# pkusys/Auncel

Measured on AMD Instinct MI355X. Metric: queries/sec @ recall@10>=0.95, SIFT-10M d=128 IVF4096, 1/2/4/8 GPU, higher is better.
Workload: dtype u8

## Files before the change

auncel_amd/build.py:

```python
import os
import subprocess

HERE = os.path.dirname(os.path.abspath(__file__))
CSRC = os.path.join(HERE, "csrc")
LIBDIR = os.path.join(HERE, "lib")
LIB = os.path.join(LIBDIR, "libauncel_amd.so")
SOURCES = ["ivf_kernels.hip", "ivf_select.hip", "ivf_filter.hip", "dataset_io.cpp", "ivf_plan.hip", "ivf_kmeans.hip", "ivf_update.hip", "ivf_subset.hip", "ivf_selector.hip", "ivf_exact.hip", "ivf_reconstruct.hip", "ivf_engine.hip"]
FLAGS = ["--offload-arch=gfx950", "-O3", "-ffp-contract=off", "-std=c++17", "-fPIC", "-shared", "-Wno-unused-result"]


LAST = {"compiled": [], "reused": 0}


def _deps(src):
    hdrs = [os.path.join(CSRC, f) for f in os.listdir(CSRC) if f.endswith(".h")]
    return [os.path.join(CSRC, src)] + hdrs + [os.path.join(HERE, "..", "include", "auncel_amd.h")]


def build(force=False):
    from concurrent.futures import ThreadPoolExecutor
    extra = os.environ.get("AUNCEL_AMD_CXXFLAGS", "").split()
    stamp = os.path.join(LIBDIR, "flags.txt")
    want = " ".join(FLAGS + extra)
    same_flags = os.path.exists(stamp) and open(stamp).read() == want
    os.makedirs(LIBDIR, exist_ok=True)
    objdir = os.path.join(LIBDIR, "obj")
    os.makedirs(objdir, exist_ok=True)
    hipcc = os.environ.get("HIPCC", "/opt/rocm/bin/hipcc")
    cflags = [f for f in FLAGS if f != "-shared"]
    todo = []
    for s in SOURCES:
        o = os.path.join(objdir, s + ".o")
        stale = force or not same_flags or not os.path.exists(o) or any(os.path.getmtime(p) > os.path.getmtime(o) for p in _deps(s))
        if stale:
            todo.append([hipcc] + cflags + extra + ["-c", os.path.join(CSRC, s), "-o", o])
    LAST["compiled"], LAST["reused"] = [os.path.basename(c[-3]) for c in todo], len(SOURCES) - len(todo)
    if not todo and os.path.exists(LIB) and same_flags:
        return LIB
    with ThreadPoolExecutor(max_workers=len(SOURCES)) as ex:
        for r in ex.map(lambda c: subprocess.run(c), todo):
            if r.returncode != 0:
                raise RuntimeError("hipcc failed")
    objs = [os.path.join(objdir, s + ".o") for s in SOURCES]
    subprocess.run([hipcc, "--offload-arch=gfx950", "-shared", "-fPIC"] + objs + ["-o", LIB], check=True)
    with open(stamp, "w") as f:
        f.write(want)
    return LIB


HOST_LIB = os.path.join(LIBDIR, "libfaiss_amd.so")
HOST_DIR = os.path.join(CSRC, "host")


def build_host(force=False):
    build(force)
    srcs = [os.path.join(HOST_DIR, f) for f in os.listdir(HOST_DIR)]
    if not force and os.path.exists(HOST_LIB) and all(os.path.getmtime(p) <= os.path.getmtime(HOST_LIB) for p in srcs + [LIB]):
        return HOST_LIB
    cmd = ["g++", "-std=c++17", "-O2", "-fPIC", "-shared", os.path.join(HOST_DIR, "faiss_amd.cpp"), "-o", HOST_LIB,
           "-L" + LIBDIR, "-launcel_amd", "-Wl,-rpath,$ORIGIN", "-pthread"]
    subprocess.run(cmd, check=True)
    return HOST_LIB


if __name__ == "__main__":
    print(build(force=True))
    print(build_host(force=True))
```

auncel_amd/csrc/ivf_engine.hip:

```cpp
#include <hip/hip_runtime.h>

#include <algorithm>
#include <atomic>
#include <cfloat>
#include <cmath>
#include <cstdlib>
#include <chrono>
#include <condition_variable>
#include <deque>
#include <functional>
#include <map>
#include <cstring>
#include <memory>
#include <stdexcept>
#include <string>
#include <mutex>
#include <thread>
#include <unordered_set>
#include <vector>

#include "../../include/auncel_amd.h"
#include "exact_args.h"
#include "ivf_kernels.h"
#include "kmeans_host.h"
// ... 1581 lines not shown
void coarse_dev(amd_ivf* h, const float* d_x, size_t n, size_t nprobe, int mode, float* d_out_dis, int64_t* d_out_keys, int fused,
                size_t prefix = 0) {
    if (!ix(h)->have_centroids) throw EngineError("quantizer has no centroids");
    const bool gemm = mode == 1 || (mode < 0 && !(n < 20 && h->d % 4 == 0));
    const size_t nlist = h->nlist;
    hipStream_t s = h->stream;
    if (!gemm && !h->in_coarse_pick && opt(h, OPT_COARSE_PICK, 2) != 0 && n >= 256 && nprobe <= 128 && nlist <= 4096 && nlist >= 4 * nprobe + 64 &&
        prefix == 0 && h->ties_override < 0 && n * nlist <= h->dist_budget_floats) {
        size_t t = h->timer.begin(CAT_COARSE, s);
        h->w_xnorms.ensure(n * sizeof(float));
        h->w_dist.ensure(n * nlist * sizeof(float));
        static const bool dbg_pick = getenv("AUNCEL_AMD_DEBUG_PICK") != nullptr;
        h->c_pick_flag.ensure((n + 1 + 8 + 8) * 4);
        h->p_pick.ensure((n + 1 + 8) * 4);
        HIP_CHECK(hipMemsetAsync(h->c_pick_flag.p, 0, 4, s));
        if (dbg_pick) HIP_CHECK(hipMemsetAsync(h->c_pick_flag.as<uint32_t>() + n + 1 + 8, 0, 32, s));
        launch_row_norms(d_x, n, h->dpad, h->w_xnorms.as<float>(), s);
        const FilterParams* prm = nullptr;
        if (opt(h, OPT_COARSE_PICK, 2) >= 2 && ix(h)->d_cinfo.p) {
            h->w_qinfo.ensure(16);
            h->w_fparams.ensure(2 * sizeof(FilterParams));
            HIP_CHECK(hipMemsetAsync(h->w_qinfo.p, 0, 16, s));
            launch_amax(d_x, n, h->dpad, h->w_qinfo.as<uint32_t>(), s);
            FilterParams* p = h->w_fparams.as<FilterParams>() + 1;
            launch_half_params(h->w_qinfo.as<uint32_t>(), ix(h)->d_cinfo.as<uint32_t>(), h->d, p, s);
            launch_coarse_gemm16(h->metric, d_x, ix(h)->d_centroids.as<float>(), h->w_xnorms.as<float>(), ix(h)->d_centroid_norms.as<float>(),
                                 (int)n, (int)nlist, h->dpad, h->w_dist.as<float>(), p, s);
            prm = p;
        } else {
            launch_coarse_gemm(h->metric, d_x, ix(h)->d_centroids.as<float>(), h->w_xnorms.as<float>(), ix(h)->d_centroid_norms.as<float>(),
                               (int)n, (int)nlist, h->dpad, h->w_dist.as<float>(), s);
        }
        launch_coarse_pick(h->metric, h->w_dist.as<float>(), d_x, ix(h)->d_centroids.as<float>(), h->w_xnorms.as<float>(), ix(h)->centroid_norm_max,
                           (uint32_t)n, (uint32_t)nlist, (uint32_t)nprobe, h->dpad, d_out_dis, d_out_keys, h->c_pick_flag.as<uint32_t>(),
                           h->c_pick_flag.as<uint32_t>() + 1, s, prm, dbg_pick ? h->c_pick_flag.as<uint32_t>() + n + 1 + 8 : nullptr);
        h->timer.end(t, s);
        CopySegs c{};
        c.src[0] = h->c_pick_flag.p;
        c.dst[0] = h->p_pick.dev();
        c.words[0] = (uint32_t)(n + 1);
        c.n = 1;
        launch_copy_segs(c, s);
        HIP_CHECK(stream_sync(s));
        const uint32_t m = h->p_pick.as<uint32_t>()[0];
        if (dbg_pick) {
            uint32_t why[5];
            HIP_CHECK(hipMemcpy(why, h->c_pick_flag.as<uint32_t>() + n + 1 + 8, sizeof(why), hipMemcpyDeviceToHost));
            fprintf(stderr, "[pick] %u of %zu rankings flagged: threshold/scale %u, too many candidates %u, too few %u, not finite %u, equal distances %u\n", m, n,
                    why[0], why[1], why[2], why[3], why[4]);
        }
        if (const uint32_t m_flagged = m) {
            const uint32_t m = (m_flagged + 7u) & ~7u;
            if (m != m_flagged) {
                uint32_t* list = h->p_pick.as<uint32_t>() + 1;
                for (uint32_t i = m_flagged; i < m; i++) list[i] = list[0];
                HIP_CHECK(hipMemcpyAsync(h->c_pick_flag.as<uint32_t>() + 1 + m_flagged, list + m_flagged, (m - m_flagged) * 4, hipMemcpyHostToDevice, s));
            }
            h->c_pick_x.ensure((size_t)m * h->dpad * sizeof(float));
            h->c_pick_dis.ensure((size_t)m * nprobe * 4);
            h->c_pick_keys.ensure((size_t)m * nprobe * 8);
            launch_gather_rows(d_x, h->c_pick_flag.as<uint32_t>() + 1, m, (uint32_t)h->dpad, h->c_pick_x.as<float>(), s);
            struct Guard {
                bool& f;
                ~Guard() { f = false; }
            } guard{h->in_coarse_pick};
            h->in_coarse_pick = true;
            coarse_dev(h, h->c_pick_x.as<float>(), m, nprobe, mode, h->c_pick_dis.as<float>(), h->c_pick_keys.as<int64_t>(), fused, 0);
            launch_scatter_rows(h->c_pick_dis.p, h->c_pick_flag.as<uint32_t>() + 1, m, (uint32_t)nprobe, d_out_dis, s);
            launch_scatter_rows(h->c_pick_keys.p, h->c_pick_flag.as<uint32_t>() + 1, m, (uint32_t)(2 * nprobe), d_out_keys, s);
        }
        h->coarse_picked = n - m;
        return;
    }
    h->coarse_picked = 0;
    const size_t chunk = std::max<size_t>(1, std::min<size_t>(n, h->dist_budget_floats / std::max<size_t>(nlist, 1)));
    const bool use_heap = nprobe <= 128;
    const int ties_opt = (int)opt(h, OPT_COARSE_TIES, -1);
    const bool heap_ties = !use_heap && (h->ties_override >= 0 ? h->ties_override == 1 : ties_opt == 1 || (ties_opt != 0 && n < 20));
    for (size_t c0 = 0; c0 < n; c0 += chunk) {
        const size_t m = std::min(chunk, n - c0);
        const uint32_t qg = scan_shape_of((uint32_t)std::min<size_t>(m, scan_qblock(false)));
        const uint32_t tv = scan_tile_vecs(qg);
        const size_t nitems = ((m + qg * SCAN_RQ - 1) / (qg * SCAN_RQ)) * ((nlist + tv - 1) / tv);
        const uint64_t csig = ((uint64_t)c0 << 40) ^ ((uint64_t)m << 20) ^ (uint64_t)nlist ^ ((uint64_t)qg << 60) ^ (use_heap ? 1ull << 59 : 0ull);
        const size_t ng = (m + SCAN_RQ - 1) / SCAN_RQ;
        const bool cached = h->coarse_sig_valid && h->coarse_sig == csig;
        if (!cached) {
            h->p_pair_query.ensure(m * 4);
            h->p_pair_out.ensure(m * 8);
            h->p_items.ensure(nitems * sizeof(ScanItem));
            h->p_group_p0.ensure(ng * 4);
            h->p_group_cnt.ensure(ng * 4);
            uint32_t* pq = h->p_pair_query.as<uint32_t>();
            uint64_t* po = h->p_pair_out.as<uint64_t>();
            ScanItem* items = h->p_items.as<ScanItem>();
            for (size_t i = 0; i < m; i++) {
                pq[i] = (uint32_t)(c0 + i);
                po[i] = (uint64_t)i * nlist;
            }
            size_t ni = 0;
            for (uint32_t vb = 0; vb < nlist; vb += tv)
                for (uint32_t qb = 0; qb < m; qb += qg * SCAN_RQ) {
                    ScanItem& it = items[ni++];
                    it.vec_base = vb;
                    it.nvec = std::min<uint32_t>(tv, (uint32_t)nlist - vb);
                    it.vec_off = vb;
                    it.pair_begin = qb;
                    it.npair = std::min<uint32_t>(qg * SCAN_RQ, (uint32_t)m - qb);
                    it.qg = qg;
                    it.qgroup = qb / SCAN_RQ;
                }
            for (size_t g = 0; g < ng; g++) {
                h->p_group_p0.as<uint32_t>()[g] = (uint32_t)(g * SCAN_RQ);
                h->p_group_cnt.as<uint32_t>()[g] = (uint32_t)std::min<size_t>(SCAN_RQ, m - g * SCAN_RQ);
            }
            h->c_pair_query.ensure(m * 4);
            h->c_pair_out.ensure(m * 8);
            h->c_items.ensure(nitems * sizeof(ScanItem));
            h->c_group_p0.ensure(ng * 4);
            h->c_group_cnt.ensure(ng * 4);
            HIP_CHECK(hipMemcpyAsync(h->c_pair_query.p, pq, m * 4, hipMemcpyHostToDevice, s));
            HIP_CHECK(hipMemcpyAsync(h->c_pair_out.p, po, m * 8, hipMemcpyHostToDevice, s));
            HIP_CHECK(hipMemcpyAsync(h->c_items.p, items, nitems * sizeof(ScanItem), hipMemcpyHostToDevice, s));
            HIP_CHECK(hipMemcpyAsync(h->c_group_p0.p, h->p_group_p0.p, ng * 4, hipMemcpyHostToDevice, s));
            HIP_CHECK(hipMemcpyAsync(h->c_group_cnt.p, h->p_group_cnt.p, ng * 4, hipMemcpyHostToDevice, s));
            h->coarse_sig_valid = false;
        }
        h->w_dist.ensure(m * nlist * sizeof(float));
        h->w_qtile.ensure(std::max<size_t>(ng, 1) * (size_t)h->dpad * SCAN_RQ * sizeof(float));
        launch_pack_queries(d_x, h->c_pair_query.as<uint32_t>(), h->c_group_p0.as<uint32_t>(), h->c_group_cnt.as<uint32_t>(), ng, h->dpad,
                            h->w_qtile.as<float>(), s);
        ScanArgs sa{};
        sa.qtile = h->w_qtile.as<float>();
        sa.codes = ix(h)->d_centroids.as<float>();
        sa.queries = d_x;
        sa.items = h->c_items.as<ScanItem>();
        sa.pair_query = h->c_pair_query.as<uint32_t>();
        sa.pair_out = h->c_pair_out.as<uint64_t>();
        sa.dist = h->w_dist.as<float>();
        sa.d = h->dpad;
        sa.metric = h->metric;
        sa.fused = fused;
        size_t t = h->timer.begin(CAT_COARSE, s);
        if (gemm) {
            h->w_xnorms.ensure(m * sizeof(float));
            launch_row_norms(d_x + c0 * h->dpad, m, h->dpad, h->w_xnorms.as<float>(), s);
            launch_coarse_gemm(h->metric, d_x + c0 * h->dpad, ix(h)->d_centroids.as<float>(), h->w_xnorms.as<float>(),
                               ix(h)->d_centroid_norms.as<float>(), (int)m, (int)nlist, h->dpad, h->w_dist.as<float>(), s);
        } else {
            size_t n_qg[4] = {0, 0, 0, 0};
            n_qg[scan_qg_class(qg)] = nitems;
            launch_scan(sa, n_qg, s);
        }
        if (use_heap) {
            const size_t k = nprobe;
            h->c_heap_val.ensure(m * k * 4);
            h->c_heap_ref.ensure(m * k * 8);
            h->c_stage.ensure(m * 4);
            h->c_nscan.ensure(m * 8);
            h->c_done.ensure(m * 4);
            h->c_seg_off.ensure(m * 8);
            h->c_seg_list.ensure(m * 4);
            h->c_seg_count.ensure(m * 4);
            constexpr size_t MISC_BYTES = STATS_ROWS * 4 * 8 + 8;
            h->w_misc.ensure(MISC_BYTES);
            if (!cached) {
                h->p_seg_off.ensure(m * 8);
                h->p_seg_list.ensure(m * 4);
                h->p_seg_count.ensure(m * 4);
                for (size_t i = 0; i < m; i++) {
                    h->p_seg_off.as<uint64_t>()[i] = (uint64_t)i * nlist;
                    h->p_seg_list.as<int32_t>()[i] = 0;
                    h->p_seg_count.as<uint32_t>()[i] = 1;
                }
                HIP_CHECK(hipMemcpyAsync(h->c_seg_off.p, h->p_seg_off.p, m * 8, hipMemcpyHostToDevice, s));
                HIP_CHECK(hipMemcpyAsync(h->c_seg_list.p, h->p_seg_list.p, m * 4, hipMemcpyHostToDevice, s));
                HIP_CHECK(hipMemcpyAsync(h->c_seg_count.p, h->p_seg_count.p, m * 4, hipMemcpyHostToDevice, s));
            }
            launch_fill_f32(h->c_heap_val.as<float>(), m * k, h->metric == METRIC_L2 ? FLT_MAX : -FLT_MAX, s);
            launch_fill_i64(h->c_heap_ref.as<int64_t>(), m * k, -1, s);
            HIP_CHECK(hipMemsetAsync(h->c_stage.p, 0, m * 4, s));
            HIP_CHECK(hipMemsetAsync(h->c_nscan.p, 0, m * 8, s));
            HIP_CHECK(hipMemsetAsync(h->c_done.p, 0, m * 4, s));
            HIP_CHECK(hipMemsetAsync(h->w_misc.p, 0, MISC_BYTES, s));
            ReplayArgs ra{};
            ra.metric = h->metric;
            ra.k = (int)k;
            ra.nlist = (uint32_t)nlist;
            ra.nq = (uint32_t)m;
            ra.round_probes = 1;
            ra.dist = h->w_dist.as<float>();
            ra.seg_off = h->c_seg_off.as<uint64_t>();
            ra.seg_list = h->c_seg_list.as<int32_t>();
            ra.seg_count = h->c_seg_count.as<uint32_t>();
            ra.identity_ids = 1;
            ra.finalize_all = 1;
            ra.heap_val = h->c_heap_val.as<float>();
            ra.heap_ref = h->c_heap_ref.as<int64_t>();
            ra.stage = h->c_stage.as<uint32_t>();
            ra.nscan = h->c_nscan.as<unsigned long long>();
            ra.done = h->c_done.as<uint32_t>();
            ra.D = d_out_dis + c0 * nprobe;
            ra.I = d_out_keys + c0 * nprobe;
            ra.stats = h->w_misc.as<unsigned long long>();
            ra.error = reinterpret_cast<uint32_t*>(h->w_misc.as<unsigned long long>() + STATS_ROWS * 4);
            launch_replay(ra, s);
        } else {
            bool tail_neutral = false;
            if (sort_rows_ranks_a_prefix((uint32_t)nlist, (uint32_t)nprobe, (uint32_t)prefix) && c0 == 0 && m == n && d_out_dis == h->w_cdis.p &&
                d_out_keys == h->w_ckeys.p) {
                amd_ivf::CoarseTail& ct = h->coarse_tail;
                tail_neutral = ct.valid && ct.dis == d_out_dis && ct.keys == d_out_keys && ct.prefix == prefix && ct.nprobe == nprobe && ct.rows >= n &&
                               ct.metric == h->metric && ct.touch_dis + 1 == h->w_cdis.touch && ct.touch_keys + 1 == h->w_ckeys.touch &&
                               !getenv("AUNCEL_AMD_WRITE_TAILS");
                ct = amd_ivf::CoarseTail{true, d_out_dis, d_out_keys, prefix, nprobe, tail_neutral ? ct.rows : n, h->metric, h->w_cdis.touch, h->w_ckeys.touch};
            } else {
                h->coarse_tail.valid = false;
            }
            launch_sort_rows(h->w_dist.as<float>(), (uint32_t)m, (uint32_t)nlist, (uint32_t)nprobe, h->metric,
                             d_out_dis + c0 * nprobe, d_out_keys + c0 * nprobe, s, (uint32_t)prefix, tail_neutral);
            if (heap_ties) {
                if (!h->w_tie_rows.p) {
                    h->w_tie_rows.ensure(8);
                    HIP_CHECK(hipMemsetAsync(h->w_tie_rows.p, 0, 8, s));
                }
                const size_t nout = prefix && prefix < nprobe ? prefix : nprobe;
                const bool ran = launch_heap_tie_order(h->w_dist.as<float>(), (uint32_t)m, (uint32_t)nlist, (uint32_t)nprobe, (uint32_t)nout,
                                                       h->metric, d_out_dis + c0 * nprobe, d_out_keys + c0 * nprobe,
                                                       h->w_tie_rows.as<unsigned long long>(), s);
                if (!ran && (h->ties_override == 1 || ties_opt == 1))
                    throw EngineError("coarse tie order by the reference's heap needs nlist x 12 bytes of LDS (nlist <= ~13 000)");
            }
        }
        h->timer.end(t, s);
        if (!cached || c0 + m < n) {
            HIP_CHECK(stream_sync(s));
            if (c0 == 0 && m == n) {
                h->coarse_sig = csig;
                h->coarse_sig_valid = true;
            }
        }
    }
}

TunerDev make_tuner(amd_ivf* h, size_t query_topk, float multipler, float std_m, const float* d_req, const float* d_gt,
                    unsigned long long* d_np, float* d_tr, int profile) {
    TunerDev t{};
    t.enabled = 1;
    t.profile = profile & 1;
    t.overhead = (profile & 2) ? 1 : 0;
    t.max_topk = (uint32_t)ix(h)->tuner_max_topk;
    t.query_topk = (uint32_t)query_topk;
    t.ntraces = (uint32_t)ix(h)->tuner_ntraces;
    t.multipler = multipler;
    t.std_m = std_m;
    t.interdis = ix(h)->d_interdis.as<float>();
    t.arcos = ix(h)->d_arcos.as<float>();
    t.trace_off = ix(h)->d_trace_off.as<uint32_t>();
    t.trace_x = ix(h)->d_trace_x.as<float>();
    t.trace_y = ix(h)->d_trace_y.as<float>();
    t.trace_std = ix(h)->d_trace_std.as<float>();
    t.require_acc = d_req;
    t.gt_D = d_gt;
    t.my_nprobe = d_np;
    t.t_recalls = d_tr;
    return t;
}

void run_rounds_device(amd_ivf* h, const RoundSpec& base, size_t n, size_t first_round_in, size_t total_nprobe,
                       const unsigned long long* d_np_abs ) {
    amd_ivf* I = ix(h);
    size_t first_round = first_round_in;
    const size_t nlist = h->nlist;
    hipStream_t s = h->stream;
    static const bool sync_env = getenv("AUNCEL_AMD_SYNC_ROUNDS") != nullptr || getenv("AUNCEL_AMD_DEBUG_REPLAY") != nullptr;
    const bool chained = !(base.range || base.d_budget_ms || sync_env);
    const double grow_env = opt(h, OPT_ROUND_GROW, 0.0);
    const bool filter_ok = filter_available(h, I, base.bytes) && !base.range;
    const bool filter_half = filter_ok && ensure_frag16(I);
    if (filter_ok && !filter_half) ensure_frag32(I);
    const float* lanes = base.bytes ? nullptr : ensure_lanes(I);
    struct Fp32Gate {
        amd_ivf* ix;
        bool held;
        Fp32Gate(amd_ivf* index, bool wanted) : ix(index), held(false) {
            if (!wanted || (int)index->opt.get(OPT_FP32_IN_FLIGHT, 4) <= 0) return;
            std::unique_lock<std::mutex> lk(ix->fp32_gate_mu);
            const uint64_t mine = ix->fp32_gate_next++;
            ix->fp32_gate_cv.wait(lk, [&] {
                const int limit = (int)ix->opt.get(OPT_FP32_IN_FLIGHT, 4);
                return mine == ix->fp32_gate_serving && (limit <= 0 || ix->fp32_running < limit);
            });
            ix->fp32_gate_serving++;
            ix->fp32_running++;
            held = true;
            lk.unlock();
            ix->fp32_gate_cv.notify_all();
        }
        ~Fp32Gate() {
            if (!held) return;
            {
                std::lock_guard<std::mutex> lk(ix->fp32_gate_mu);
                ix->fp32_running--;
            }
            ix->fp32_gate_cv.notify_all();
        }
    } fp32_gate(I, !base.bytes && n >= 256);
    if (filter_ok && base.tuner.enabled) first_round = filter_first_probes(I, (size_t)base.k, 64, 0.015);
    const double grow = grow_env > 0 ? grow_env : base.bytes ? 12.0 : filter_ok ? 6.0 : 3.5;
    size_t seg_cap = (size_t)2 << 20;
    if (!base.bytes) {
        const size_t groups = ((size_t)4 << 30) / ((size_t)h->dpad * SCAN_RQ * sizeof(float));
        seg_cap = std::min(seg_cap, std::max<size_t>((size_t)64 << 10, (groups > nlist ? groups - nlist : 0) * SCAN_RQ));
    }
    size_t maxlist = 0;
    for (size_t l = 0; l < nlist; l++) maxlist = std::max<size_t>(maxlist, I->h_list_off[l + 1] - I->h_list_off[l]);
    const size_t item_cap = (seg_cap / 32 + nlist) * ((maxlist + SCAN_WAVE_VECS - 1) / SCAN_WAVE_VECS) + nlist * 4 + 16;
    static const size_t seg_cap_env = getenv("AUNCEL_AMD_SEG_CAP_PAIRS") ? (size_t)atol(getenv("AUNCEL_AMD_SEG_CAP_PAIRS")) : 0;
// ... 1685 lines not shown
        const bool can_spec = !no_spec && h->spec_wanted && !h->given_keys && np_row == nlist && n <= h->dist_budget_floats / std::max<size_t>(nlist, 1) &&
                              heap_tie_order_lds((uint32_t)nlist, (uint32_t)nlist) <= 160 * 1024;
        if (!can_spec && !fuse_small)
            launch_first_tie(h->w_cdis.as<float>(), (uint32_t)n, (uint32_t)nlist, (uint32_t)h->first_tie_nreal, h->w_first_tie.as<uint32_t>(), h->stream);
        if (can_spec) {
            const size_t ncopy = std::min(h->first_tie_nreal, nlist);
            h->w_spec_full.ensure((size_t)SPEC_CAP * nlist * 4);
            h->w_spec_dis.ensure((size_t)SPEC_CAP * nlist * 4);
            h->w_spec_keys.ensure((size_t)SPEC_CAP * nlist * 8);
            h->w_spec_count.ensure(32);
            h->w_spec_slot.ensure(n * 4);
            h->w_spec_query.ensure((size_t)SPEC_CAP * 4);
            ensure_context_streams(h);
            HIP_CHECK(hipStreamWaitEvent(h->stream, h->ev_spec_done, 0));
            HIP_CHECK(hipMemsetAsync(h->w_spec_count.p, 0, 32, h->stream));
            (void)SPEC_NEAR;
            launch_tie_collect(h->w_cdis.as<float>(), (uint32_t)n, (uint32_t)h->first_tie_nreal, SPEC_WINDOW, SPEC_CAP, (uint32_t)nlist, (uint32_t)ncopy,
                               h->w_dist.as<float>(), h->w_ckeys.as<int64_t>(), h->w_first_tie.as<uint32_t>(), h->w_spec_count.as<uint32_t>(),
                               h->w_spec_slot.as<int32_t>(), h->w_spec_full.as<float>(), h->w_spec_dis.as<float>(), h->w_spec_keys.as<int64_t>(),
                               h->w_spec_query.as<uint32_t>(), h->stream);
            HIP_CHECK(hipEventRecord(h->ev_spec_go, h->stream));
            HIP_CHECK(hipStreamWaitEvent(h->spec_stream, h->ev_spec_go, 0));
            launch_heap_tie_order(h->w_spec_full.as<float>(), SPEC_CAP, (uint32_t)nlist, (uint32_t)nlist, (uint32_t)ncopy, h->metric,
                                  h->w_spec_dis.as<float>(), h->w_spec_keys.as<int64_t>(),
                                  reinterpret_cast<unsigned long long*>(h->w_spec_count.as<uint32_t>() + 2), h->spec_stream,
                                  h->w_spec_count.as<uint32_t>());
            HIP_CHECK(hipEventRecord(h->ev_spec_done, h->spec_stream));
            h->spec_valid = true;
            h->spec_ncopy = ncopy;
            static const bool no_patch = getenv("AUNCEL_AMD_NO_TIE_PATCH") != nullptr;
            h->spec_inline = !no_patch && (nlist & (nlist - 1)) == 0 && nlist >= 64;
        }
    }
    const bool tie_inline = h->want_first_tie && h->spec_valid && h->spec_inline;
    struct FuseScope {
        amd_ivf* h;
        bool on;
        FuseScope(amd_ivf* hh, bool o) : h(hh), on(o) {
            if (on) {
                h->fuse = amd_ivf::SmallFuse{};
                h->fuse.active = true;
            }
        }
        ~FuseScope() { h->fuse.active = false; }
    } fuse_scope(h, fuse_small);
    init_state(h, n, K, true);
    auto set_online = [h, nlist, n, np_row](const uint32_t* only = nullptr, const uint32_t* only_count = nullptr, uint32_t cap = 0) {
        launch_set_online(h->metric, (uint32_t)nlist, only ? cap : (uint32_t)n, h->w_cdis.as<float>(), h->w_ckeys.as<int64_t>(), (uint32_t)np_row,
                          ix(h)->d_interdis.as<float>(), ix(h)->d_arcos.as<float>(), h->w_dtb.as<float>(), h->w_error.as<uint32_t>(), h->stream,
                          only, only_count);
    };
    if (!fuse_small && !tie_inline) set_online();
    RoundSpec base;
    if (tie_inline) {
        size_t maxlist = 0;
        for (size_t l = 0; l < nlist; l++) maxlist = std::max<size_t>(maxlist, ix(h)->h_list_off[l + 1] - ix(h)->h_list_off[l]);
        const size_t SCRATCH_FLOATS = std::min<size_t>((size_t)64 << 20, std::max<size_t>((size_t)8 << 20, (size_t)h->spec_cap * 16 * ((maxlist + 1023) & ~(size_t)1023)));
        h->w_spec_scratch.ensure(SCRATCH_FLOATS * 4);
        base.run_ties = true;
        base.before_first_select = [h, nlist, set_online, SCRATCH_FLOATS]() {
            HIP_CHECK(hipStreamWaitEvent(h->stream, h->ev_spec_done, 0));
            TiePatchArgs ta{};
            ta.count = h->w_spec_count.as<uint32_t>();
            ta.cap = h->spec_cap;
            ta.nlist = (uint32_t)nlist;
            ta.ncopy = (uint32_t)h->spec_ncopy;
            ta.key_stride = (uint32_t)nlist;
            ta.slot_query = h->w_spec_query.as<uint32_t>();
            ta.slot_of = h->w_spec_slot.as<int32_t>();
            ta.s_keys = h->w_spec_keys.as<int64_t>();
            ta.ckeys = h->w_ckeys.as<int64_t>();
            ta.seg_count = h->w_pl_cnt.as<uint32_t>();
            ta.seg_begin = h->w_seg_begin.as<uint32_t>();
            ta.seg_list = h->w_seg_list.as<int32_t>();
            ta.seg_off = h->w_seg_off.as<uint64_t>();
            ta.list_off = ix(h)->d_list_off.as<uint64_t>();
            ta.dist = h->w_dist.as<float>();
            ta.row_align = h->row_align_now;
            ta.scratch = h->w_spec_scratch.as<float>();
            ta.scratch_floats = SCRATCH_FLOATS;
            ta.cursor = reinterpret_cast<unsigned long long*>(h->w_spec_count.as<uint32_t>() + 4);
            ta.patched = h->w_spec_count.as<uint32_t>() + 1;
            launch_tie_patch(ta, h->stream);
            set_online();
        };
        static const bool no_split = getenv("AUNCEL_AMD_NO_SPLIT_SELECT") != nullptr;
        if (!no_split && n >= 256) {
            h->w_split.ensure((2 * n + 8) * 4);
            uint32_t* counts = h->w_split.as<uint32_t>();
            uint32_t* q_free = counts + 8;
            uint32_t* q_wait = q_free + n;
            const auto patch_hook = base.before_first_select;
            const uint32_t wait_cap = (uint32_t)std::min<size_t>(n, h->spec_cap);
            base.split_free = q_free;
            base.split_wait = q_wait;
            base.split_counts = counts;
            base.split_wait_cap = wait_cap;
            base.split_prepare = [h, n, counts, q_free, q_wait, set_online]() {
                HIP_CHECK(hipMemsetAsync(counts, 0, 8, h->stream));
                launch_partition_qsel(nullptr, nullptr, (uint32_t)n, h->w_spec_slot.as<int32_t>(), q_free, q_wait, counts, h->stream);
                set_online();
            };
            base.split_between = [h, patch_hook, counts, q_wait, wait_cap, set_online]() {
                (void)set_online;
                patch_hook();
            };
        }
    }
    base.fused = ix(h)->allow_fused && ix(h)->db_range.fusable_with(qr, h->metric);
    base.bytes = byte_queries(h, ix(h), d_x, n, qr);
    if (fuse_small) {
        h->fuse.active = false;
        SmallStateArgs sa{};
        sa.init = h->fuse.init;
        sa.metric = h->metric;
        sa.nlist = (uint32_t)nlist;
        sa.nq = (uint32_t)n;
        sa.coarse_dis = h->w_cdis.as<float>();
        sa.coarse_keys = h->w_ckeys.as<int64_t>();
        sa.coarse_stride = (uint32_t)np_row;
        sa.interdis = ix(h)->d_interdis.as<float>();
        sa.arcos = ix(h)->d_arcos.as<float>();
        sa.dtb = h->w_dtb.as<float>();
        if (h->want_first_tie) {
            sa.ft_sorted_dis = h->w_cdis.as<float>();
            sa.ft_stride = (uint32_t)nlist;
            sa.ft_nreal = (uint32_t)h->first_tie_nreal;
            sa.ft_out = h->w_first_tie.as<uint32_t>();
        }
        if (h->fuse.have_bytes) {
            sa.bx = h->fuse.bx;
            sa.bout = h->fuse.bout;
            sa.bcx = h->fuse.bcx;
        }
        sa.d = h->d;
        sa.dpad = h->dpad;
        launch_small_state(sa, h->stream);
    }
    ix(h)->last_arith = base.bytes ? 2 : base.fused ? 1 : 0;
    base.k = (int)K;
    base.id_offset = start;
    base.d_x = d_x;
    base.d_cdis = h->w_cdis.as<float>();
    base.d_ckeys = h->w_ckeys.as<int64_t>();
    base.coarse_stride = (uint32_t)np_row;
    base.tuner = make_tuner(h, query_topk, multipler, std_m, dreq, dgt, dnp, dtr, profile);
    const size_t first_env = std::max<size_t>(1, (size_t)opt(h, OPT_ROUND_FIRST, 12));
    base.caller_checks_error = true;
    DirectOut direct(h, D, I);
    host_stamp("state");
    if (n < 20)
        base.spec_finish = [&]() {
            finish_results(h, n, K, D, I, nullptr, true);
            tail_gathers();
        };
    run_rounds_device(h, base, n, first_env, np_row, dnp);
    host_stamp("rounds");
    if (!h->spec_done) {
        finish_results(h, n, K, D, I, nullptr, true);
        tail_gathers();
        sync_and_flush(h, h->stream);
    }
    h->spec_done = false;
    host_stamp("final-sync");
    const double wall = wc.stop();
    host_stamp("clock");
    print_stamps();
    double ms[NCAT], ln[NCAT];
    h->timer.collect(ms, NCAT, ln);
    fill_timing(h, ms, ln);
    h->timer.off = false;
    h->timing[3] = wall;
    h->timing[5] = h->scan_bytes;
    h->last_min_bytes = h->scan_min_bytes;
    h->timing[6] = h->scan_slots > 0 ? h->scan_useful / h->scan_slots : 0;
}

static void adaptive_redo_ties(amd_ivf_t* h, const float* d_x, size_t start, size_t n, size_t query_topk, float multipler, float std_m,
                               const float* require_acc, const float* gt_D, int profile, int coarse_mode, uint64_t* my_nprobe,
                               float* t_recalls, float* D, int64_t* I, const IntRange& qr) {
    const size_t K = ix(h)->tuner_max_topk, nlist = h->nlist;
    const std::vector<uint64_t> np0(my_nprobe + start, my_nprobe + start + n);
    const std::vector<float> tr0(t_recalls + start, t_recalls + start + n);
    const size_t nreal = std::min(coarse_read_bound(nlist, multipler, np0.data(), n), nlist);
    TieRegime regime(h);
    h->ties_override = 0;
    h->want_first_tie = true;
    h->first_tie_nreal = nreal;
// ... 2458 lines not shown
```

auncel_amd/csrc/ivf_kernels.h:

```cpp
#pragma once
#include <hip/hip_runtime.h>
#include <stddef.h>
#include <stdint.h>
#include <stdio.h>
#include <stdlib.h>
#include <string.h>

#include <stdexcept>
#include <string>

#include "selector_args.h"

namespace amdivf {

inline void check_launch(const char* what) {
    const hipError_t e = hipGetLastError();
    if (e != hipSuccess) throw std::runtime_error(std::string("kernel launch failed: ") + what + ": " + hipGetErrorString(e));
    static const bool sync_each = getenv("AUNCEL_AMD_SYNC_LAUNCH") != nullptr;
    if (sync_each) {
        fprintf(stderr, "[launch] %.100s\n", what);
        const hipError_t s = hipDeviceSynchronize();
        if (s != hipSuccess) throw std::runtime_error(std::string("kernel failed: ") + what + ": " + hipGetErrorString(s));
    }
}
#define LAUNCH(...)                     \
    do {                                \
        (void)hipGetLastError();        \
        hipLaunchKernelGGL(__VA_ARGS__); \
        ::amdivf::check_launch(#__VA_ARGS__); \
    } while (0)

constexpr int METRIC_IP = 0;
constexpr int METRIC_L2 = 1;

constexpr int SCAN_RQ = 8;
constexpr int SCAN_RV = 2;
#ifndef AUNCEL_SCAN_DC
#define AUNCEL_SCAN_DC 16
#endif
constexpr int SCAN_DC = AUNCEL_SCAN_DC;
constexpr int SCAN_WAVE_VECS = 64 * SCAN_RV;

constexpr int SCAN_VB_BITS = 40;
constexpr uint64_t SCAN_VB_MASK = (1ull << SCAN_VB_BITS) - 1;
inline __host__ __device__ uint64_t scan_vec_base(uint64_t first_vector, uint64_t first_block32_of_list, uint32_t pos_in_list) {
    return first_vector | (((first_block32_of_list >> 1) + pos_in_list / 64u) << SCAN_VB_BITS);
}

struct ScanItem {
    uint64_t vec_base;
    uint32_t nvec;
    uint32_t vec_off;
    uint32_t pair_begin;
    uint32_t npair;
    uint32_t qg;
    uint32_t qgroup;
};

struct ScanArgs {
    const float* codes;
    const float* queries;
    const ScanItem* items;
    const uint32_t* pair_query;
    const uint64_t* pair_out;
    float* dist;
    const float* qtile;
    int d;
    int metric;
    int fused;
    const float* thr;
    unsigned long long* mask;
    int xcd_chunks;
    uint32_t nitems;
    const uint32_t* dev_counts;
    uint32_t hint_qg[4];
    int hint_valid;
    const float* lanes;
};

void launch_scan(const ScanArgs& a, const size_t n_qg[4], hipStream_t s, hipStream_t s2 = nullptr, hipStream_t s1 = nullptr,
                 hipStream_t s4 = nullptr);
void launch_lanes_from_f32(const float* codes, const uint64_t* list_off, const uint64_t* block_off, uint32_t nlist, uint64_t nblocks64, int dpad,
                           float* out, hipStream_t s);
constexpr int CNT_ACTIVE = 0, CNT_SEGMENTS = 1, CNT_PAIRS = 2, CNT_GROUPS = 3, CNT_QG1 = 4, CNT_QG2 = 5, CNT_QG4 = 8, CNT_QG8 = 9;
unsigned resident_grid(unsigned workgroups_per_cu);

void launch_pack_queries(const float* queries, const uint32_t* pair_query, const uint32_t* group_p0, const uint32_t* group_cnt,
                         size_t ngroups, int d, float* qtile, hipStream_t s, const uint32_t* dev_ngroups = nullptr, uint32_t hint = 0);

constexpr uint32_t MFMA_BLOCK = 32;
constexpr uint32_t MFMA_QBLOCK = 32;
uint32_t mfma_chunk();
uint32_t mfma_chunk_thr();
inline __host__ __device__ uint32_t mfma_ksteps(int d) { return (uint32_t)(d + 31) / 32; }
inline __host__ __device__ uint64_t mfma_list_blocks(uint64_t size) { return ((size + 63) / 64) * 2; }

struct MfmaScanArgs {
    const uint8_t* codes_frag;
    const int32_t* code_cy;
    const int8_t* queries8;
    const int32_t* query_cx;
    const ScanItem* items;
    const uint32_t* pair_query;
    const uint64_t* pair_out;
    float* dist;
    const float* thr;
    unsigned long long* mask;
    int d;
    int metric;
    int xcd_chunks;
    uint32_t nitems;
    const uint32_t* dev_nitems;
    uint32_t hint_nitems;
    int debug;
    int exact_mask;
    int pipelined;
};
void launch_scan_mfma(const MfmaScanArgs& a, hipStream_t s);
uint32_t mfma_thr_qblock(int d, int pipelined, bool exact_mask);
void launch_frag_from_f32(const float* codes, const uint64_t* list_off, const uint64_t* block_off, uint32_t nlist, uint64_t nblocks, int d,
                          int dpad, int metric, uint8_t* out, int32_t* cy, hipStream_t s);
void launch_sbytes_from_f32(const float* x, size_t n, int d, int dpad, int metric, int8_t* out, int32_t* cx, hipStream_t s);
inline __host__ __device__ uint32_t filter_steps(int d) {
    const uint32_t j = (uint32_t)(d + 7) / 8;
    return j <= 4 ? 4u : j <= 8 ? 8u : j <= 12 ? 12u : j <= 16 ? 16u : (j + 1u) & ~1u;
}
struct FilterScanArgs {
    const float* codes_frag;
    const float* yn;
    const float* xf;
    const float* xn;
    const float* codes;
    const float* queries;
    const ScanItem* items;
    const uint32_t* pair_query;
    const uint64_t* pair_out;
    float* dist;
    const float* thr;
    unsigned long long* mask;
    uint4* surv;
    uint32_t* surv_count;
    uint32_t surv_cap;
    int d, dpad;
    int metric;
    int xcd_chunks;
    uint32_t nitems;
    const uint32_t* dev_nitems;
    uint32_t hint_nitems;
    int half;
    const float* params;
};
struct FilterParams {
    float sx, ps, C, pad;
};
struct KeepArgs;
struct KeepEachArgs;
void launch_scan_filter(const FilterScanArgs& a, hipStream_t s, const KeepArgs* keep = nullptr, const KeepEachArgs* keep_each = nullptr);
inline __host__ __device__ uint32_t filter_steps16(int d) {
    const uint32_t j = (uint32_t)(d + 15) / 16;
    return j <= 4 ? 4u : j <= 6 ? 6u : j <= 8 ? 8u : (j + 1u) & ~1u;
}
void launch_amax(const float* x, size_t rows, int stride, uint32_t* info, hipStream_t s);
float filter_half_scale(const uint32_t info[4], int d);
void launch_half_params(const uint32_t* qinfo, const uint32_t* yinfo, int d, FilterParams* params, hipStream_t s);
void launch_frag16_from_f32(const float* codes, const uint64_t* list_off, const uint64_t* block_off, uint32_t nlist, uint64_t nblocks, int d,
                            int dpad, int metric, const uint32_t* info, float* out, float* yn, hipStream_t s);
void launch_filter_queries16(const float* x, size_t n, int d, int dpad, int metric, const uint32_t* qinfo, const uint32_t* yinfo, float* xf,
                             float* xn, FilterParams* params, hipStream_t s);
constexpr uint32_t FILTER_WIDE_QUERIES = 128;
constexpr uint32_t FILTER_WIDE_VECTORS = 128;
uint32_t filter_item_queries(int d);
// ... 556 lines not shown
```

Measured before the change: 2.882 million.

## Add direct register-tiled exact coarse distance kernel bypassing scan staging

```diff
diff --git a/auncel_amd/build.py b/auncel_amd/build.py
--- a/auncel_amd/build.py
+++ b/auncel_amd/build.py
@@ -5,7 +5,7 @@
 CSRC = os.path.join(HERE, "csrc")
 LIBDIR = os.path.join(HERE, "lib")
 LIB = os.path.join(LIBDIR, "libauncel_amd.so")
-SOURCES = ["ivf_kernels.hip", "ivf_select.hip", "ivf_filter.hip", "dataset_io.cpp", "ivf_plan.hip", "ivf_kmeans.hip", "ivf_update.hip", "ivf_subset.hip", "ivf_selector.hip", "ivf_exact.hip", "ivf_reconstruct.hip", "ivf_engine.hip"]
+SOURCES = ["ivf_kernels.hip", "ivf_coarse.hip", "ivf_select.hip", "ivf_filter.hip", "dataset_io.cpp", "ivf_plan.hip", "ivf_kmeans.hip", "ivf_update.hip", "ivf_subset.hip", "ivf_selector.hip", "ivf_exact.hip", "ivf_reconstruct.hip", "ivf_engine.hip"]
 FLAGS = ["--offload-arch=gfx950", "-O3", "-ffp-contract=off", "-std=c++17", "-fPIC", "-shared", "-Wno-unused-result"]
 
 
diff --git a/auncel_amd/csrc/ivf_coarse.hip b/auncel_amd/csrc/ivf_coarse.hip
--- /dev/null
+++ b/auncel_amd/csrc/ivf_coarse.hip
@@ -0,0 +1,152 @@
+#include "ivf_dev.h"
+
+#include <algorithm>
+
+#pragma clang fp contract(off)
+
+namespace amdivf {
+
+constexpr int COARSE_RQ = 4;
+constexpr int COARSE_RV = 4;
+constexpr int COARSE_WAVES = 8;
+constexpr int COARSE_NT = COARSE_WAVES * 64;
+constexpr int COARSE_TQ = COARSE_WAVES * COARSE_RQ;
+constexpr int COARSE_TC = 64 * COARSE_RV;
+constexpr int COARSE_DC = 16;
+constexpr int COARSE_SLOTS = COARSE_DC / 4;
+constexpr int COARSE_ROW = COARSE_DC + 4;
+constexpr int COARSE_NLD = COARSE_TC * COARSE_SLOTS / COARSE_NT;
+static_assert(COARSE_TC * COARSE_SLOTS % COARSE_NT == 0, "tile must split evenly over the workgroup");
+
+typedef float cf2 __attribute__((ext_vector_type(2)));
+typedef float cv4f __attribute__((ext_vector_type(4)));
+typedef const cv4f __attribute__((address_space(4)))* coarse_const_f4p;
+
+template <int METRIC>
+__global__ __launch_bounds__(COARSE_NT) __attribute__((amdgpu_waves_per_eu(4, 4)))
+void coarse_exact_kernel(const float* __restrict__ x, const float* __restrict__ cen, uint32_t n, uint32_t nlist, int d, uint32_t ctiles,
+                         float* __restrict__ out) {
+    __shared__ float lds[2][COARSE_TC * COARSE_ROW];
+    const int tid = threadIdx.x;
+    const int lane = tid & 63;
+    const int wave = __builtin_amdgcn_readfirstlane(tid >> 6);
+    const uint32_t ct = blockIdx.x % ctiles, qb = blockIdx.x / ctiles;
+    const uint32_t c0 = ct * COARSE_TC;
+    const uint32_t q0 = qb * COARSE_TQ + (uint32_t)wave * COARSE_RQ;
+    const bool has_queries = q0 < n;
+
+    coarse_const_f4p qrow[COARSE_RQ];
+#pragma unroll
+    for (int r = 0; r < COARSE_RQ; r++) {
+        const uint32_t q = q0 + r < n ? q0 + r : n - 1;
+        qrow[r] = (coarse_const_f4p)(uintptr_t)(x + (size_t)q * (size_t)d);
+    }
+
+    cf2 acc[COARSE_RQ][COARSE_RV][2];
+#pragma unroll
+    for (int r = 0; r < COARSE_RQ; r++)
+#pragma unroll
+        for (int v = 0; v < COARSE_RV; v++) acc[r][v][0] = acc[r][v][1] = cf2{0.f, 0.f};
+
+    const float* tile_base = cen + (size_t)c0 * (size_t)d;
+    const uint32_t nrows = nlist - c0 < (uint32_t)COARSE_TC ? nlist - c0 : (uint32_t)COARSE_TC;
+    float4 pre[COARSE_NLD];
+    auto fetch = [&](int cc) {
+#pragma unroll
+        for (int i = 0; i < COARSE_NLD; i++) {
+            const int idx = tid + i * COARSE_NT;
+            const int row = idx / COARSE_SLOTS, slot = idx % COARSE_SLOTS;
+            pre[i] = make_float4(0.f, 0.f, 0.f, 0.f);
+            if ((uint32_t)row < nrows && cc + slot * 4 < d) pre[i] = *reinterpret_cast<const float4*>(tile_base + (size_t)row * d + cc + slot * 4);
+        }
+    };
+
+    const int nsteps = d >> 2;
+    cv4f qn[COARSE_RQ];
+#pragma unroll
+    for (int r = 0; r < COARSE_RQ; r++) qn[r] = *qrow[r];
+
+    fetch(0);
+    int buf = 0;
+    for (int cc = 0; cc < d; cc += COARSE_DC, buf ^= 1) {
+        float* stage = lds[buf];
+#pragma unroll
+        for (int i = 0; i < COARSE_NLD; i++) {
+            const int idx = tid + i * COARSE_NT;
+            *reinterpret_cast<float4*>(&stage[(idx / COARSE_SLOTS) * COARSE_ROW + (idx % COARSE_SLOTS) * 4]) = pre[i];
+        }
+        __syncthreads();
+        if (cc + COARSE_DC < d) fetch(cc + COARSE_DC);
+        if (!has_queries) continue;
+        const int nslot = (d - cc >= COARSE_DC ? COARSE_DC : d - cc) >> 2;
+        const float* myrow = &stage[lane * COARSE_ROW];
+        float4 yn[COARSE_RV];
+#pragma unroll
+        for (int v = 0; v < COARSE_RV; v++) yn[v] = *reinterpret_cast<const float4*>(myrow + v * 64 * COARSE_ROW);
+#pragma unroll
+        for (int s = 0; s < COARSE_SLOTS; s++) {
+            if (s >= nslot) break;
+            const int t = (cc >> 2) + s;
+            cv4f qc[COARSE_RQ];
+            cf2 ya[COARSE_RV], yb[COARSE_RV];
+#pragma unroll
+            for (int r = 0; r < COARSE_RQ; r++) qc[r] = qn[r];
+#pragma unroll
+            for (int v = 0; v < COARSE_RV; v++) {
+                ya[v] = cf2{yn[v].x, yn[v].y};
+                yb[v] = cf2{yn[v].z, yn[v].w};
+            }
+            if (t + 1 < nsteps) {
+#pragma unroll
+                for (int r = 0; r < COARSE_RQ; r++) qn[r] = *(qrow[r] + (t + 1));
+            }
+            if (s + 1 < nslot) {
+#pragma unroll
+                for (int v = 0; v < COARSE_RV; v++) yn[v] = *reinterpret_cast<const float4*>(myrow + v * 64 * COARSE_ROW + (s + 1) * 4);
+            }
+#pragma unroll
+            for (int r = 0; r < COARSE_RQ; r++) {
+                const cf2 qa = cf2{qc[r].x, qc[r].y}, qb2 = cf2{qc[r].z, qc[r].w};
+#pragma unroll
+                for (int v = 0; v < COARSE_RV; v++) {
+                    if (METRIC == METRIC_L2) {
+                        const cf2 ta = ya[v] - qa, tb = yb[v] - qb2;
+                        acc[r][v][0] += ta * ta;
+                        acc[r][v][1] += tb * tb;
+                    } else {
+                        acc[r][v][0] += ya[v] * qa;
+                        acc[r][v][1] += yb[v] * qb2;
+                    }
+                }
+            }
+        }
+    }
+
+    if (!has_queries) return;
+#pragma unroll
+    for (int r = 0; r < COARSE_RQ; r++) {
+        if (q0 + r >= n) break;
+        float* orow = out + (size_t)(q0 + r) * (size_t)nlist + c0;
+#pragma unroll
+        for (int v = 0; v < COARSE_RV; v++) {
+            const uint32_t c = (uint32_t)(v * 64 + lane);
+            const float res = (acc[r][v][0].x + acc[r][v][0].y) + (acc[r][v][1].x + acc[r][v][1].y);
+            if (c < nrows) orow[c] = res;
+        }
+    }
+}
+
+void launch_coarse_exact(int metric, const float* x, const float* centroids, size_t n, size_t nlist, int dpad, float* dist, hipStream_t s) {
+    if (n == 0 || nlist == 0) return;
+    const size_t ctiles = (nlist + COARSE_TC - 1) / COARSE_TC, qblocks = (n + COARSE_TQ - 1) / COARSE_TQ;
+    const dim3 grid((unsigned)(ctiles * qblocks)), block(COARSE_NT);
+    if (metric == METRIC_L2) LAUNCH(coarse_exact_kernel<METRIC_L2>, grid, block, 0, s, x, centroids, (uint32_t)n, (uint32_t)nlist, dpad, (uint32_t)ctiles, dist);
+    else LAUNCH(coarse_exact_kernel<METRIC_IP>, grid, block, 0, s, x, centroids, (uint32_t)n, (uint32_t)nlist, dpad, (uint32_t)ctiles, dist);
+}
+
+bool coarse_exact_covers(size_t n, size_t nlist, int dpad) {
+    const size_t ctiles = (nlist + COARSE_TC - 1) / COARSE_TC, qblocks = (n + COARSE_TQ - 1) / COARSE_TQ;
+    return dpad > 0 && dpad % 4 == 0 && n < (1ull << 32) && nlist < (1ull << 32) && ctiles * qblocks < (1ull << 31);
+}
+
+}
diff --git a/auncel_amd/csrc/ivf_engine.hip b/auncel_amd/csrc/ivf_engine.hip
--- a/auncel_amd/csrc/ivf_engine.hip
+++ b/auncel_amd/csrc/ivf_engine.hip
@@ -1687,10 +1687,13 @@
         const uint32_t qg = scan_shape_of((uint32_t)std::min<size_t>(m, scan_qblock(false)));
         const uint32_t tv = scan_tile_vecs(qg);
         const size_t nitems = ((m + qg * SCAN_RQ - 1) / (qg * SCAN_RQ)) * ((nlist + tv - 1) / tv);
-        const uint64_t csig = ((uint64_t)c0 << 40) ^ ((uint64_t)m << 20) ^ (uint64_t)nlist ^ ((uint64_t)qg << 60) ^ (use_heap ? 1ull << 59 : 0ull);
+        const bool direct = !gemm && m == n && coarse_exact_covers(m, nlist, h->dpad);
+        const uint64_t csig = ((uint64_t)c0 << 40) ^ ((uint64_t)m << 20) ^ (uint64_t)nlist ^ ((uint64_t)qg << 60) ^ (use_heap ? 1ull << 59 : 0ull) ^
+                              (direct ? 1ull << 58 : 0ull);
         const size_t ng = (m + SCAN_RQ - 1) / SCAN_RQ;
-        const bool cached = h->coarse_sig_valid && h->coarse_sig == csig;
-        if (!cached) {
+        const bool staged = !direct || use_heap;
+        const bool cached = staged && h->coarse_sig_valid && h->coarse_sig == csig;
+        if (!cached && !direct) {
             h->p_pair_query.ensure(m * 4);
             h->p_pair_out.ensure(m * 8);
             h->p_items.ensure(nitems * sizeof(ScanItem));
@@ -1732,9 +1735,11 @@
             h->coarse_sig_valid = false;
         }
         h->w_dist.ensure(m * nlist * sizeof(float));
-        h->w_qtile.ensure(std::max<size_t>(ng, 1) * (size_t)h->dpad * SCAN_RQ * sizeof(float));
-        launch_pack_queries(d_x, h->c_pair_query.as<uint32_t>(), h->c_group_p0.as<uint32_t>(), h->c_group_cnt.as<uint32_t>(), ng, h->dpad,
-                            h->w_qtile.as<float>(), s);
+        if (!direct) {
+            h->w_qtile.ensure(std::max<size_t>(ng, 1) * (size_t)h->dpad * SCAN_RQ * sizeof(float));
+            launch_pack_queries(d_x, h->c_pair_query.as<uint32_t>(), h->c_group_p0.as<uint32_t>(), h->c_group_cnt.as<uint32_t>(), ng, h->dpad,
+                                h->w_qtile.as<float>(), s);
+        }
         ScanArgs sa{};
         sa.qtile = h->w_qtile.as<float>();
         sa.codes = ix(h)->d_centroids.as<float>();
@@ -1752,6 +1757,8 @@
             launch_row_norms(d_x + c0 * h->dpad, m, h->dpad, h->w_xnorms.as<float>(), s);
             launch_coarse_gemm(h->metric, d_x + c0 * h->dpad, ix(h)->d_centroids.as<float>(), h->w_xnorms.as<float>(),
                                ix(h)->d_centroid_norms.as<float>(), (int)m, (int)nlist, h->dpad, h->w_dist.as<float>(), s);
+        } else if (direct) {
+            launch_coarse_exact(h->metric, d_x, ix(h)->d_centroids.as<float>(), m, nlist, h->dpad, h->w_dist.as<float>(), s);
         } else {
             size_t n_qg[4] = {0, 0, 0, 0};
             n_qg[scan_qg_class(qg)] = nitems;
@@ -1838,7 +1845,7 @@
             }
         }
         h->timer.end(t, s);
-        if (!cached || c0 + m < n) {
+        if (staged && (!cached || c0 + m < n)) {
             HIP_CHECK(stream_sync(s));
             if (c0 == 0 && m == n) {
                 h->coarse_sig = csig;
@@ -3690,6 +3697,10 @@
             ta.cursor = reinterpret_cast<unsigned long long*>(h->w_spec_count.as<uint32_t>() + 4);
             ta.patched = h->w_spec_count.as<uint32_t>() + 1;
             launch_tie_patch(ta, h->stream);
+        };
+        const auto tie_patch = base.before_first_select;
+        base.before_first_select = [tie_patch, set_online]() {
+            tie_patch();
             set_online();
         };
         static const bool no_split = getenv("AUNCEL_AMD_NO_SPLIT_SELECT") != nullptr;
@@ -3698,7 +3709,6 @@
             uint32_t* counts = h->w_split.as<uint32_t>();
             uint32_t* q_free = counts + 8;
             uint32_t* q_wait = q_free + n;
-            const auto patch_hook = base.before_first_select;
             const uint32_t wait_cap = (uint32_t)std::min<size_t>(n, h->spec_cap);
             base.split_free = q_free;
             base.split_wait = q_wait;
@@ -3709,9 +3719,9 @@
                 launch_partition_qsel(nullptr, nullptr, (uint32_t)n, h->w_spec_slot.as<int32_t>(), q_free, q_wait, counts, h->stream);
                 set_online();
             };
-            base.split_between = [h, patch_hook, counts, q_wait, wait_cap, set_online]() {
-                (void)set_online;
-                patch_hook();
+            base.split_between = [h, tie_patch, set_online]() {
+                tie_patch();
+                set_online(h->w_spec_query.as<uint32_t>(), h->w_spec_count.as<uint32_t>(), h->spec_cap);
             };
         }
     }
diff --git a/auncel_amd/csrc/ivf_kernels.h b/auncel_amd/csrc/ivf_kernels.h
--- a/auncel_amd/csrc/ivf_kernels.h
+++ b/auncel_amd/csrc/ivf_kernels.h
@@ -87,6 +87,9 @@
 
 void launch_pack_queries(const float* queries, const uint32_t* pair_query, const uint32_t* group_p0, const uint32_t* group_cnt,
                          size_t ngroups, int d, float* qtile, hipStream_t s, const uint32_t* dev_ngroups = nullptr, uint32_t hint = 0);
+
+void launch_coarse_exact(int metric, const float* x, const float* centroids, size_t n, size_t nlist, int dpad, float* dist, hipStream_t s);
+bool coarse_exact_covers(size_t n, size_t nlist, int dpad);
 
 constexpr uint32_t MFMA_BLOCK = 32;
 constexpr uint32_t MFMA_QBLOCK = 32;
```

Result: slower. 2.844 million (-1.3%).
